# oviniciuscesar/Pseudo-Quadrature-Mirror-Filter

Measured on NVIDIA B200. Metric: PQMF analyze+inverse throughput (n_band=16), higher is better.
Workload: dtype f32

## Files before the change

pseudo-quadrature-mirror-filter_b200/csrc/hankel4.cuh:

```cuda
#pragma once
#include <cuda_fp16.h>
#include <cuda_runtime.h>
#include <math.h>
#include <stdint.h>
#include <string.h>

#include <atomic>

#include "half_io.cuh"
#include "hankel16.cuh"
#include "pcm.cuh"
#include "ptx.cuh"

namespace pqmf {

constexpr int kH4Workers = 256;
constexpr int kH4Threads = kH4Workers + 32;
constexpr int kH4SynWorkers = 288;
constexpr int kH4SynThreads = kH4SynWorkers + 32;
constexpr int kH4Rows = 128;
constexpr int kH4TileSamples = 64 * kH4Rows;
constexpr int kH4MaxPlaneRows = 144;
constexpr float kH4Res = 2048.0f;

__device__ __forceinline__ uint64_t umma_desc_sw128(uint32_t smem_addr) {
  uint64_t d = 0;
  d |= (uint64_t)((smem_addr & 0x3FFFFu) >> 4);
  d |= (uint64_t)1 << 16;
  d |= (uint64_t)(1024u >> 4) << 32;
  d |= (uint64_t)1 << 46;
  d |= (uint64_t)2 << 61;
  return d;
}
__device__ __forceinline__ uint32_t sw128_offset(uint32_t byte_lin) { return byte_lin ^ (((byte_lin >> 7) & 7u) << 4); }

struct H4Shape {
  int jlo, kt, ks;
  int rows, plane;
  int bank;
  int bytes;
// ... 37 lines not shown
}

__device__ __forceinline__ void split2_f16s(float a, float b, uint32_t& h1_bits, uint32_t& h2_bits) {
  const __half2 h1 = __floats2half2_rn(a, b);
  const float2 h1f = __half22float2(h1);
  const float2 r = __ffma2_rn(h1f, make_float2(-kH4Res, -kH4Res), __fmul2_rn(make_float2(a, b), make_float2(kH4Res, kH4Res)));
  const __half2 h2 = __floats2half2_rn(r.x, r.y);
  h1_bits = *reinterpret_cast<const uint32_t*>(&h1);
  h2_bits = *reinterpret_cast<const uint32_t*>(&h2);
}
__device__ __forceinline__ float2 h4_combine2(uint32_t d0a, uint32_t d0b, uint32_t d1a, uint32_t d1b) {
  const float2 t = __ffma2_rn(make_float2(__uint_as_float(d1a), __uint_as_float(d1b)), make_float2(1.0f / kH4Res, 1.0f / kH4Res),
                              make_float2(__uint_as_float(d0a), __uint_as_float(d0b)));
  constexpr float kInv = 1.0f / (float)(1 << kH16ScaleLog2);
  return __fmul2_rn(t, make_float2(kInv, kInv));
}

template <int N>
__device__ __forceinline__ void h4_tmem_ld(uint32_t taddr, uint32_t (&r)[N]) {
  static_assert(N == 2 || N == 4 || N == 8 || N == 16 || N == 32, "columns per load");
  if constexpr (N == 2) ptx::tmem_ld2(taddr, r);
  else if constexpr (N == 4) ptx::tmem_ld4(taddr, r);
  else if constexpr (N == 8) ptx::tmem_ld8(taddr, r);
  else if constexpr (N == 16) ptx::tmem_ld16(taddr, r);
  else ptx::tmem_ld32(taddr, r);
}

#ifdef PQMF_H4_TRACE
#define H4_STAMP(k) do { if (blockIdx.x == 0 && (tid & 31) == 0 && it < 64) p.trace[((size_t)it * 8 + warp) * 8 + (k)] = clock64(); } while (0)
#else
#define H4_STAMP(k) do { } while (0)
#endif

struct H4Smem {
  unsigned char *bank, *planes;
  uint64_t *pfull, *mma_bar, *bankfull;
  uint32_t* tmem_slot;
};
__device__ __forceinline__ H4Smem h4_carve(unsigned char* smem, const H4Shape& g) {
  H4Smem s;
  s.bank = smem;
  s.planes = smem + g.bank;
  s.pfull = reinterpret_cast<uint64_t*>(smem + g.bank + 4 * g.plane);
  s.mma_bar = s.pfull + 2;
  s.bankfull = s.mma_bar + 2;
  s.tmem_slot = reinterpret_cast<uint32_t*>(s.bankfull + 1);
  return s;
}

template <bool PAIR>
__device__ __forceinline__ uint32_t h4_prologue(const H4Smem& s, const H4Shape& g, const uint16_t* bank_images, uint32_t rank, int worker_warps,
                                                int tid) {
  const int warp = tid >> 5;
  ptx::grid_dep_launch();
  if (tid == 0) {
    for (int i = 0; i < 2; ++i) {
      ptx::mbar_init(&s.pfull[i], worker_warps * (PAIR ? 2 : 1));
      ptx::mbar_init(&s.mma_bar[i], 1);
    }
    ptx::mbar_init(s.bankfull, 1);
    ptx::fence_barrier_init();
    ptx::mbar_arrive_expect_tx(s.bankfull, (uint32_t)g.bank);
    ptx::bulk_g2s(s.bank, reinterpret_cast<const unsigned char*>(bank_images) + (size_t)rank * g.bank, (uint32_t)g.bank, s.bankfull);
  }
  if (warp == 0) {
    if constexpr (PAIR) {
      ptx::tmem_alloc_pair(s.tmem_slot, 256);
    } else {
      ptx::tmem_alloc(s.tmem_slot, 256);
      ptx::tmem_relinquish();
    }
  }
  ptx::tc_fence_before();
  __syncthreads();
  if constexpr (PAIR) ptx::cluster_sync_all();
  ptx::tc_fence_after();
  ptx::grid_dep_wait();
  return *s.tmem_slot;
}

template <bool PAIR>
__device__ __forceinline__ void h4_teardown(uint32_t tmem, int warp) {
  ptx::tc_fence_before();
  __syncthreads();
  if constexpr (PAIR) {
    ptx::cluster_sync_all();
    if (warp == 0) ptx::tmem_dealloc_pair(tmem, 256);
  } else {
    if (warp == 0) ptx::tmem_dealloc(tmem, 256);
  }
}

template <bool PAIR>
__device__ __forceinline__ void h4_issuer_loop(const H4Smem& s, const H4Shape& g, uint32_t tmem, unsigned n_iter, int pad_bytes, int tlo,
                                               int thi, unsigned it0 = 0) {
  const uint32_t bank_addr = ptx::smem_u32(s.bank), plane_addr = ptx::smem_u32(s.planes);
  for (unsigned it = it0; it < it0 + n_iter; ++it) {
    const int pb = (int)(it & 1);
    ptx::mbar_wait(&s.pfull[pb], (it >> 1) & 1);
    ptx::tc_fence_after();
    if (ptx::elect_one_sync()) {
      h4_issue_mmas<PAIR>(tmem + (uint32_t)(pb * 128), plane_addr + (2 * pb) * g.plane, plane_addr + (2 * pb + 1) * g.plane, bank_addr, g.ks,
                          pad_bytes, tlo, thi);
      if constexpr (PAIR) ptx::umma_pair_commit(&s.mma_bar[pb]);
      else ptx::umma_commit(&s.mma_bar[pb]);
    }
    __syncwarp();
  }
}

template <bool PAIR>
__device__ __forceinline__ void h4_publish(const H4Smem& s, uint32_t pfull_leader, unsigned it, int pb, int tid, unsigned it0 = 0, unsigned bank_phase = 0) {
  ptx::fence_proxy_async();
  ptx::tc_fence_before();
  __syncwarp();
  if ((tid & 31) == 0) {
    if (it == it0) ptx::mbar_wait(s.bankfull, bank_phase & 1);
    if constexpr (PAIR) ptx::mbar_arrive_cluster(pfull_leader + 8u * pb);
    else ptx::mbar_arrive(&s.pfull[pb]);
  }
}

struct H4AnalysisParams {
  const float* x;
  PcmIn in;
  float* y;
  const uint16_t* bank;
  long T, F;
  int off;
  int parity;
  int trim_lo, trim_hi;
  int accumulate;
  int keep_in_l2;
  H4Shape g;
  long tiles_per_row, n_tiles;
#ifdef PQMF_H4_TRACE
  long long* trace;
#endif
};

template <int M, bool PAIR, H4Io IO>
__global__ void __launch_bounds__(kH4Threads, 1) h4_analysis_kernel(H4AnalysisParams p) {
  constexpr bool PCM = IO == H4Io::PCM, HALF = h4_io_half(IO);
  constexpr int FR = 64 / M;
  constexpr int HB = M / 2;
  constexpr int NO = (kH4MaxPlaneRows * 8 + kH4Workers - 1) / kH4Workers;
  extern __shared__ __align__(1024) unsigned char h4_smem[];
  const H4Shape g = p.g;
  const H4Smem sm = h4_carve(h4_smem, g);
  const int tid = threadIdx.x, warp = tid >> 5;
  constexpr int kMmaWarp = kH4Workers / 32;
  const uint32_t rank = PAIR ? ptx::cluster_ctarank() : 0u;
  const uint32_t tmem = h4_prologue<PAIR>(sm, g, p.bank, rank, kH4Workers / 32, tid);
  const uint32_t pfull_leader = PAIR ? ptx::mapa_shared(ptx::smem_u32(sm.pfull), 0) : 0u;

  const unsigned tpr = (unsigned)p.tiles_per_row;
  const unsigned step_b = gridDim.x / tpr, step_c = gridDim.x % tpr;
  unsigned b = blockIdx.x / tpr, c = blockIdx.x % tpr;
  const unsigned first_tile = PAIR ? (blockIdx.x & ~1u) : blockIdx.x;
  const unsigned n_iter = (unsigned)((p.n_tiles - first_tile + gridDim.x - 1) / gridDim.x);
  const unsigned n_rows = (unsigned)(p.n_tiles / p.tiles_per_row);
#ifdef PQMF_H4_TRACE
  long long cta_c0 = clock64(), cta_t0;
  asm volatile("mov.u64 %0, %%globaltimer;" : "=l"(cta_t0));
#endif

  if (warp == kMmaWarp) {
    if (rank == 0) h4_issuer_loop<PAIR>(sm, g, tmem, n_iter, 0, p.trim_lo, p.trim_hi);
  } else {
    const int n_octs = g.rows * 8;
    float x0[NO][8];
    auto load_window = [&](unsigned bb, unsigned cc) {
      const long s0 = (long)cc * kH4TileSamples + g.jlo - p.off;
      const float* xrow = p.x + (size_t)bb * p.T;
      const uint16_t* xhrow = reinterpret_cast<const uint16_t*>(p.x) + (size_t)bb * p.T;
#pragma unroll
      for (int r = 0; r < NO; ++r) {
        const int o = tid + kH4Workers * r;
        const long s = s0 + 8L * o;
        if (bb < n_rows && o < n_octs && s >= 0 && s < p.T) {
          if constexpr (PCM) {
            pcm_load8_raw(p.in, bb, s, p.T, x0[r]);
          } else if constexpr (HALF) {
            const float4 raw = ptx::ldg128_na(reinterpret_cast<const float4*>(xhrow + s));
            x0[r][0] = raw.x; x0[r][1] = raw.y; x0[r][2] = raw.z; x0[r][3] = raw.w;
          } else {
            ptx::ldg256_na(xrow + s, x0[r]);
          }
        } else {
#pragma unroll
          for (int e = 0; e < 8; ++e) x0[r][e] = 0.f;
        }
      }
    };
    auto convert = [&](int pb, unsigned bb, unsigned cc) {
      unsigned char* p1 = sm.planes + (2 * pb) * g.plane;
      unsigned char* p2 = p1 + g.plane;
#pragma unroll
      for (int r = 0; r < NO; ++r) {
        const int o = tid + kH4Workers * r;
        if (o < n_octs) {
          if constexpr (PCM) {
            const long s = (long)cc * kH4TileSamples + g.jlo - p.off + 8L * o;
            if (bb < n_rows && s >= 0 && s < p.T) pcm_convert8(p.in, bb, x0[r]);
          }
          if constexpr (HALF) h4_widen8<IO>(x0[r]);
          uint4 a, bq;
          split2_f16s(x0[r][0], x0[r][1], a.x, bq.x);
          split2_f16s(x0[r][2], x0[r][3], a.y, bq.y);
          split2_f16s(x0[r][4], x0[r][5], a.z, bq.z);
          split2_f16s(x0[r][6], x0[r][7], a.w, bq.w);
          const uint32_t off = sw128_offset((uint32_t)o * 16u);
          *reinterpret_cast<uint4*>(p1 + off) = a;
          *reinterpret_cast<uint4*>(p2 + off) = bq;
        }
      }
    };
    auto advance = [&](unsigned& bb, unsigned& cc) {
      bb += step_b;
      cc += step_c;
      if (cc >= tpr) {
        cc -= tpr;
        ++bb;
      }
    };
    auto epilogue = [&](unsigned bb, unsigned cc, int dbuf) {
      const int i = tid & 127, hb = tid >> 7;
      const uint32_t taddr = tmem + ((uint32_t)((warp & 3) * 32) << 16) + (uint32_t)(dbuf * 128 + HB * hb);
      const long n = ((long)cc * kH4Rows + i) * FR;
      uint32_t r0[FR][HB], r1[FR][HB];
#pragma unroll
      for (int dl = 0; dl < FR; ++dl) {
        h4_tmem_ld<HB>(taddr + dl * M, r0[dl]);
        h4_tmem_ld<HB>(taddr + 64 + dl * M, r1[dl]);
      }
      ptx::tmem_ld_wait();
      float v[FR][HB];
#pragma unroll
      for (int dl = 0; dl < FR; ++dl) {
        const uint32_t flip = (((FR > 1 ? dl : (int)(n & 1)) + p.parity) & 1) == 0 ? 0x80000000u : 0u;
#pragma unroll
        for (int kk = 0; kk < HB; kk += 2) {
          const float2 t = h4_combine2(r0[dl][kk], r0[dl][kk + 1], r1[dl][kk], r1[dl][kk + 1]);
          v[dl][kk] = t.x;
          v[dl][kk + 1] = __uint_as_float(__float_as_uint(t.y) ^ flip);
        }
      }
      if constexpr (HALF) {
        uint16_t* yp = reinterpret_cast<uint16_t*>(p.y) + ((size_t)bb * M + HB * hb) * p.F + n;
        if (n + FR - 1 < p.F && (p.F % (FR >= 8 ? 8 : FR)) == 0) {
#pragma unroll
          for (int kk = 0; kk < HB; ++kk) {
            uint16_t* q = yp + (size_t)kk * p.F;
            if constexpr (FR >= 8) {
#pragma unroll
              for (int d8 = 0; d8 < FR; d8 += 8) {
// ... 29 lines not shown
          for (int kk = 0; kk < HB; ++kk)
#pragma unroll
            for (int dl = 0; dl < FR; ++dl) prev[dl][kk] = __ldcs(yp + (size_t)kk * p.F + dl);
#pragma unroll
          for (int kk = 0; kk < HB; ++kk)
#pragma unroll
            for (int dl = 0; dl < FR; ++dl) v[dl][kk] += prev[dl][kk];
        }
#pragma unroll
        for (int kk = 0; kk < HB; ++kk) {
          float* q = yp + (size_t)kk * p.F;
          if constexpr (FR >= 4) {
#pragma unroll
            for (int d4 = 0; d4 < FR; d4 += 4) {
              const float4 w = make_float4(v[d4][kk], v[d4 + 1][kk], v[d4 + 2][kk], v[d4 + 3][kk]);
              if (p.keep_in_l2) *reinterpret_cast<float4*>(q + d4) = w;
              else __stcs(reinterpret_cast<float4*>(q + d4), w);
            }
          } else if constexpr (FR == 2) {
            __stcs(reinterpret_cast<float2*>(q), make_float2(v[0][kk], v[1][kk]));
          } else {
            __stcs(q, v[0][kk]);
          }
        }
      } else {
#pragma unroll
        for (int kk = 0; kk < HB; ++kk)
#pragma unroll
          for (int dl = 0; dl < FR; ++dl)
            if (n + dl < p.F) yp[(size_t)kk * p.F + dl] = v[dl][kk] + (p.accumulate ? yp[(size_t)kk * p.F + dl] : 0.f);
      }
    };

    unsigned b1 = b, c1 = c;
    advance(b1, c1);
    load_window(b, c);
    unsigned prev_b = 0, prev_c = 0;
    for (unsigned it = 0; it < n_iter; ++it) {
      const int pb = (int)(it & 1);
      H4_STAMP(0);
      convert(pb, b, c);
      H4_STAMP(1);
      h4_publish<PAIR>(sm, pfull_leader, it, pb, tid);
      if (it + 1 < n_iter) load_window(b1, c1);
      H4_STAMP(2);
      if (it > 0) {
        ptx::mbar_wait(&sm.mma_bar[(it - 1) & 1], ((it - 1) >> 1) & 1);
        ptx::tc_fence_after();
        if (prev_b < n_rows) epilogue(prev_b, prev_c, (int)((it - 1) & 1));
      }
      H4_STAMP(5);
      prev_b = b;
      prev_c = c;
      b = b1;
      c = c1;
      advance(b1, c1);
    }
    ptx::mbar_wait(&sm.mma_bar[(n_iter - 1) & 1], ((n_iter - 1) >> 1) & 1);
    ptx::tc_fence_after();
    if (prev_b < n_rows) epilogue(prev_b, prev_c, (int)((n_iter - 1) & 1));
  }
#ifdef PQMF_H4_TRACE
  __syncthreads();
  if (tid == 0) {
    long long t1;
    asm volatile("mov.u64 %0, %%globaltimer;" : "=l"(t1));
    p.trace[64 * 64 + 2 * blockIdx.x] = clock64() - cta_c0;
    p.trace[64 * 64 + 2 * blockIdx.x + 1] = t1 - cta_t0;
  }
#endif
  h4_teardown<PAIR>(tmem, warp);
}

struct H4SynthesisParams {
  const float* s;
  float* out;
  int16_t* pcm_out;
  int C;
  int duo;
  const uint16_t* bank;
  long F;
  int o;
  int parity;
  int trim_lo, trim_hi;
  int accumulate;
  int reverse;
  H4Shape g;
  long tiles_per_row, n_tiles;
#ifdef PQMF_H4_TRACE
  long long* trace;
#endif
};

template <int M, bool PAIR, H4Io IO>
__global__ void __launch_bounds__(kH4SynThreads, 1) h4_synthesis_kernel(H4SynthesisParams p) {
  constexpr bool PCM = IO == H4Io::PCM, HALF = h4_io_half(IO);
  constexpr int FR = 64 / M;
  constexpr int NBG = M >= 8 ? M / 8 : 1;
  constexpr int FPI = M >= 8 ? 4 : 32 / M;
  extern __shared__ __align__(1024) unsigned char h4s_smem[];
  const H4Shape g = p.g;
  const H4Smem sm = h4_carve(h4s_smem, g);
  const int tid = threadIdx.x, warp = tid >> 5;
  constexpr int kMmaWarp = kH4SynWorkers / 32;
  const uint32_t rank = PAIR ? ptx::cluster_ctarank() : 0u;
  const uint32_t tmem = h4_prologue<PAIR>(sm, g, p.bank, rank, kH4SynWorkers / 32, tid);
  const uint32_t pfull_leader = PAIR ? ptx::mapa_shared(ptx::smem_u32(sm.pfull), 0) : 0u;

  const unsigned tpr = (unsigned)p.tiles_per_row;
  const unsigned step_b = gridDim.x / tpr, step_c = gridDim.x % tpr;
  unsigned b = blockIdx.x / tpr, c = blockIdx.x % tpr;
  const unsigned first_tile = PAIR ? (blockIdx.x & ~1u) : blockIdx.x;
  const unsigned G = (PCM && p.duo) ? 2u : 1u;
  const unsigned n_iter = G * (unsigned)((p.n_tiles - first_tile + gridDim.x - 1) / gridDim.x);
  const unsigned n_rows = (unsigned)(p.n_tiles / p.tiles_per_row);

  const int ehi = (g.jlo + g.kt) / M - 1;
  const int pad = (p.o - ehi) & 3;
  const int nbase = p.o - ehi - pad;
  if (warp == kMmaWarp) {
    if (rank == 0) h4_issuer_loop<PAIR>(sm, g, tmem, n_iter, 2 * M * pad, p.trim_lo, p.trim_hi);
  } else {
    const int n_fq = (g.rows * FR + FPI - 1) / FPI;
    const int bg = tid / n_fq, fq = tid - bg * n_fq;
    const bool has_item = tid < n_fq * NBG;
    float4 v0[8];
    auto load4h = [&](const uint16_t* at, bool ok) {
      if (!ok) return make_float4(0.f, 0.f, 0.f, 0.f);
      const float2 raw = ptx::ldg64_na(at);
      return make_float4(raw.x, raw.y, 0.f, 0.f);
    };
    auto load_frames = [&](float4 (&v)[8], unsigned bb, unsigned cc, unsigned hh) {
      if (p.reverse && bb < n_rows) {
        bb = n_rows - 1 - bb;
        cc = tpr - 1 - cc;
      }
      const long n = (long)cc * (kH4Rows * FR) + nbase + FPI * fq;
      const bool live = bb < n_rows && has_item;
      const size_t row = (size_t)bb * G + hh;
      if constexpr (HALF) {
        if constexpr (M >= 8) {
          const uint16_t* sp = reinterpret_cast<const uint16_t*>(p.s) + (row * M + 8 * bg) * p.F + n;
          const bool ok = live && n >= 0 && n + 3 < p.F;
#pragma unroll
          for (int kk = 0; kk < 8; ++kk) v[kk] = load4h(sp + (size_t)kk * p.F, ok);
        } else {
          const uint16_t* sp = reinterpret_cast<const uint16_t*>(p.s) + row * M * p.F + n;
#pragma unroll
          for (int kk = 0; kk < 8; ++kk) {
            const int b4 = kk >> 1, h = kk & 1;
            v[kk] = load4h(sp + (size_t)b4 * p.F + 4 * h, live && n + 4 * h >= 0 && n + 4 * h + 3 < p.F);
          }
        }
      } else if constexpr (M >= 8) {
        const float* sp = p.s + (row * M + 8 * bg) * p.F + n;
        const bool ok = live && n >= 0 && n + 3 < p.F;
#pragma unroll
        for (int kk = 0; kk < 8; ++kk) v[kk] = ok ? ptx::ldg128_na(reinterpret_cast<const float4*>(sp + (size_t)kk * p.F)) : make_float4(0.f, 0.f, 0.f, 0.f);
      } else {
        const float* sp = p.s + row * M * p.F + n;
#pragma unroll
        for (int kk = 0; kk < 8; ++kk) {
          const int b4 = kk >> 1, h = kk & 1;
          const bool ok = live && n + 4 * h >= 0 && n + 4 * h + 3 < p.F;
          v[kk] = ok ? ptx::ldg128_na(reinterpret_cast<const float4*>(sp + (size_t)b4 * p.F + 4 * h)) : make_float4(0.f, 0.f, 0.f, 0.f);
        }
      }
    };
    const uint32_t flip_even = (p.parity & 1) ? 0u : 0x80000000u, flip_odd = flip_even ^ 0x80000000u;
    auto advance = [&](unsigned& bb, unsigned& cc) {
      bb += step_b;
      cc += step_c;
      if (cc >= tpr) {
        cc -= tpr;
        ++bb;
      }
    };
    auto convert = [&](const float4 (&v)[8], int pb) {
      if (!has_item) return;
      unsigned char* p1 = sm.planes + (2 * pb) * g.plane;
      auto comp = [](const float4& q, int c) { return c == 0 ? q.x : c == 1 ? q.y : c == 2 ? q.z : q.w; };
#pragma unroll
      for (int j = 0; j < 4; ++j) {
        float w[8];
        uint32_t o;
        if constexpr (M >= 8) {
          const uint32_t fl = (j & 1) ? flip_odd : flip_even;
#pragma unroll
          for (int kk = 0; kk < 8; ++kk) {
            const float t = comp(v[kk], j);
            w[kk] = (kk & 1) ? __uint_as_float(__float_as_uint(t) ^ fl) : t;
          }
          o = sw128_offset((uint32_t)(4 * fq + j) * (2u * M) + 16u * bg);
        } else {
#pragma unroll
          for (int kk = 0; kk < 8; ++kk) {
            const int b4 = kk & 3, odd = kk >> 2;
            const float t = comp(v[2 * b4 + (j >> 1)], 2 * (j & 1) + odd);
            w[kk] = (b4 & 1) ? __uint_as_float(__float_as_uint(t) ^ (odd ? flip_odd : flip_even)) : t;
          }
          o = sw128_offset((uint32_t)(8 * fq + 2 * j) * (2u * M));
        }
        uint4 h1, h2;
        split2_f16s(w[0], w[1], h1.x, h2.x);
        split2_f16s(w[2], w[3], h1.y, h2.y);
        split2_f16s(w[4], w[5], h1.z, h2.z);
        split2_f16s(w[6], w[7], h1.w, h2.w);
        *reinterpret_cast<uint4*>(p1 + o) = h1;
        *reinterpret_cast<uint4*>(p1 + g.plane + o) = h2;
      }
// ... 65 lines not shown
          }
          return;
        }
#pragma unroll
        for (int q = 0; q < 4; ++q)
          if (t0 + 64 * q + 7 < total) pcm_store8(p.pcm_out, p.C, (long)row, t0 + 64 * q, total, val[q]);
        return;
      }
      if constexpr (HALF) {
        uint16_t* op = reinterpret_cast<uint16_t*>(p.out) + row * total + t0;
#pragma unroll
        for (int q = 0; q < 4; ++q)
          if (t0 + 64 * q + 7 < total) {
            const uint4 w = make_uint4(h4_narrow2<IO>(val[q][0], val[q][1]), h4_narrow2<IO>(val[q][2], val[q][3]), h4_narrow2<IO>(val[q][4], val[q][5]),
                                       h4_narrow2<IO>(val[q][6], val[q][7]));
            __stcs(reinterpret_cast<uint4*>(op + (size_t)q * 64), w);
          }
        return;
      }
      float* op = p.out + row * total + t0;
#pragma unroll
      for (int q = 0; q < 4; ++q)
        if (t0 + 64 * q + 7 < total) {
          if (p.accumulate) {
            float prev[8];
            ptx::ldg256_cs(op + (size_t)q * 64, prev);
#pragma unroll
            for (int e = 0; e < 8; ++e) val[q][e] += prev[e];
          }
          ptx::stg256_cs(op + (size_t)q * 64, val[q]);
        }
    };

    auto next_visit = [&](unsigned& bb, unsigned& cc, unsigned& hh) {
      if (++hh == G) {
        hh = 0;
        advance(bb, cc);
      }
    };
    unsigned h = 0, b1 = b, c1 = c, h1 = 0;
    next_visit(b1, c1, h1);
    load_frames(v0, b, c, h);
    unsigned prev_b = 0, prev_c = 0, prev_h = 0;
    for (unsigned it = 0; it < n_iter; ++it) {
      const int pb = (int)(it & 1);
      H4_STAMP(0);
      if constexpr (HALF) {
        float4 w[8];
#pragma unroll
        for (int kk = 0; kk < 8; ++kk) w[kk] = h4_widen4<IO>(v0[kk]);
        convert(w, pb);
      } else {
        convert(v0, pb);
      }
      H4_STAMP(1);
      h4_publish<PAIR>(sm, pfull_leader, it, pb, tid);
      if (it + 1 < n_iter) load_frames(v0, b1, c1, h1);
      H4_STAMP(2);
      if (it > 0) {
        ptx::mbar_wait(&sm.mma_bar[(it - 1) & 1], ((it - 1) >> 1) & 1);
        ptx::tc_fence_after();
        if (warp < 8 && prev_b < n_rows) epilogue(prev_b, prev_c, prev_h, (int)((it - 1) & 1));
      }
      H4_STAMP(5);
      prev_b = b;
      prev_c = c;
      prev_h = h;
      b = b1;
      c = c1;
      h = h1;
      next_visit(b1, c1, h1);
    }
    ptx::mbar_wait(&sm.mma_bar[(n_iter - 1) & 1], ((n_iter - 1) >> 1) & 1);
    ptx::tc_fence_after();
    if (warp < 8 && prev_b < n_rows) epilogue(prev_b, prev_c, prev_h, (int)((n_iter - 1) & 1));
  }
  h4_teardown<PAIR>(tmem, warp);
}

struct H4Configured {
  std::atomic<int> bytes[64];
  H4Configured() {
    for (auto& b : bytes) b.store(0, std::memory_order_relaxed);
  }
};
inline int h4_sm_count(int dev) {
  static std::atomic<int> sm_count[64];
  int n = sm_count[dev].load(std::memory_order_relaxed);
  if (n == 0) {
    cudaDeviceGetAttribute(&n, cudaDevAttrMultiProcessorCount, dev);
    n = n > 0 ? n : 148;
    sm_count[dev].store(n, std::memory_order_relaxed);
  }
  return n;
}
template <typename Kern>
inline int h4_configure(Kern kern, int bytes, H4Configured& configured, int& sm_count_out) {
  int dev = 0;
  cudaGetDevice(&dev);
  dev &= 63;
  if (configured.bytes[dev].load(std::memory_order_acquire) < bytes) {
    cudaError_t e = cudaFuncSetAttribute(kern, cudaFuncAttributeMaxDynamicSharedMemorySize, bytes);
    if (e != cudaSuccess) return (int)e;
    int seen = configured.bytes[dev].load(std::memory_order_relaxed);
    while (seen < bytes && !configured.bytes[dev].compare_exchange_weak(seen, bytes, std::memory_order_release)) {
    }
  }
  sm_count_out = h4_sm_count(dev);
  return 0;
}

template <bool PAIR, typename Kern, typename Params>
inline int h4_launch(Kern kern, Params p, int B, long row_samples, int threads, H4Configured& configured, cudaStream_t st) {
  int sms = 0;
  if (!h4_shape_fits(p.g)) return -2;
  if (int e = h4_configure(kern, p.g.bytes, configured, sms)) return e;
  p.tiles_per_row = (row_samples + kH4TileSamples - 1) / kH4TileSamples;
  p.n_tiles = p.tiles_per_row * B;
  if (p.tiles_per_row >= (1L << 31) || p.n_tiles >= (1L << 40)) return -2;
  long grid = PAIR ? (sms & ~1) : sms;
  const long want = PAIR ? ((p.n_tiles + 1) & ~1L) : p.n_tiles;
  if (grid > want) grid = want;
  if constexpr (PAIR) {
    cudaLaunchConfig_t cfg = {};
    cfg.gridDim = dim3((unsigned)grid);
    cfg.blockDim = dim3((unsigned)threads);
    cfg.dynamicSmemBytes = (size_t)p.g.bytes;
    cfg.stream = st;
    cudaLaunchAttribute attr[2];
    attr[0].id = cudaLaunchAttributeClusterDimension;
    attr[0].val.clusterDim.x = 2;
    attr[0].val.clusterDim.y = 1;
    attr[0].val.clusterDim.z = 1;
    attr[1].id = cudaLaunchAttributeProgrammaticStreamSerialization;
    attr[1].val.programmaticStreamSerializationAllowed = 1;
    cfg.attrs = attr;
    cfg.numAttrs = 2;
    return (int)cudaLaunchKernelEx(&cfg, kern, p);
  } else {
    kern<<<(unsigned)grid, threads, p.g.bytes, st>>>(p);
    return (int)cudaGetLastError();
  }
}

template <int M, bool PAIR>
int h4_launch_analysis(H4AnalysisParams p, int B, cudaStream_t st, H4Io io = H4Io::F32) {
  static H4Configured configured[4];
  if (p.in.pcm != nullptr) io = H4Io::PCM;
  if (io != H4Io::F32) {
    if constexpr (PAIR) {
      switch (io) {
        case H4Io::PCM: return h4_launch<PAIR>(h4_analysis_kernel<M, PAIR, H4Io::PCM>, p, B, p.F * M, kH4Threads, configured[1], st);
        case H4Io::F16: return h4_launch<PAIR>(h4_analysis_kernel<M, PAIR, H4Io::F16>, p, B, p.F * M, kH4Threads, configured[2], st);
        case H4Io::BF16: return h4_launch<PAIR>(h4_analysis_kernel<M, PAIR, H4Io::BF16>, p, B, p.F * M, kH4Threads, configured[3], st);
        default: return -2;
      }
    } else {
      return -2;
    }
  }
  return h4_launch<PAIR>(h4_analysis_kernel<M, PAIR, H4Io::F32>, p, B, p.F * M, kH4Threads, configured[0], st);
}

template <int M, bool PAIR>
int h4_launch_synthesis(H4SynthesisParams p, int B, cudaStream_t st, H4Io io = H4Io::F32) {
  static H4Configured configured[4];
  if (p.pcm_out != nullptr) {
    if constexpr (PAIR) {
      p.duo = (p.C == 2 && B % 2 == 0) ? 1 : 0;
      return h4_launch<PAIR>(h4_synthesis_kernel<M, PAIR, H4Io::PCM>, p, p.duo ? B / 2 : B, p.F * M, kH4SynThreads, configured[1], st);
    } else {
      return -2;
    }
  }
  if (h4_io_half(io)) {
    if constexpr (PAIR) {
      if (io == H4Io::F16) return h4_launch<PAIR>(h4_synthesis_kernel<M, PAIR, H4Io::F16>, p, B, p.F * M, kH4SynThreads, configured[2], st);
      return h4_launch<PAIR>(h4_synthesis_kernel<M, PAIR, H4Io::BF16>, p, B, p.F * M, kH4SynThreads, configured[3], st);
    } else {
      return -2;
    }
  }
  return h4_launch<PAIR>(h4_synthesis_kernel<M, PAIR, H4Io::F32>, p, B, p.F * M, kH4SynThreads, configured[0], st);
}

inline void hankel4_build_banks(const float* hk , int M, int L, int jlo, int kt, uint16_t* img_analysis, uint16_t* img_synthesis) {
  auto bits = [](float v) {
    const __half h = __float2half_rn(v);
    uint16_t u;
    memcpy(&u, &h, 2);
    return u;
  };
  const int ks = (kt + 64 - M + 15) / 16, kp = 16 * ks;
  const int elo = jlo / M, ehi = (jlo + kt) / M - 1;
  const float sa = (float)(1 << kH16ScaleLog2), ss = (float)M * sa;
  for (int kc = 0; kc < kp / 8; ++kc)
    for (int row = 0; row < 128; ++row)
      for (int e8 = 0; e8 < 8; ++e8) {
        const int kap = 8 * kc + e8;
// ... 59 lines not shown
```

pseudo-quadrature-mirror-filter_b200/csrc/pqmf_b200.cu:

```cuda
#include "../../include/pqmf_b200.h"

#include <cuda_fp16.h>
#include <cuda_runtime.h>

#include <atomic>
#include <cmath>
#include <cstdio>
#include <cstdlib>
#include <cstring>
#include <mutex>
#include <thread>
#include <vector>

#include "direct_form.cuh"
#include "fast16.cuh"
#include "fast16_synth.cuh"
#include "hankel16.cuh"
#include "hankel4.cuh"
#include "hankel4_stream.cuh"

namespace {

std::atomic<unsigned long long> g_launches{0};

// ... 503 lines not shown
    }
    if (rc) break;
    check(cudaEventRecord(ws.kdone[slot], ks));
    prev.live = true;
    prev.slot = slot;
    prev.r0 = r0;
    prev.n = n;
  }
  if (prev.live && rc == PQMF_OK) copy_out(prev, ws.kst[prev.slot]);
  for (int i = 0; i < kHostSlots; ++i) {
    check(cudaStreamSynchronize(ws.st[i]));
    check(cudaStreamSynchronize(ws.kst[i]));
  }
  return rc;
}

}

extern "C" {

int pqmf_abi_version(void) { return PQMF_B200_ABI_VERSION; }

const char* pqmf_strerror(int code) {
  switch (code) {
    case PQMF_OK: return "ok";
    case PQMF_ERR_ARG: return "pqmf_b200: invalid argument (null pointer, bad size or misaligned buffer)";
    case PQMF_ERR_UNSUPPORTED: return "pqmf_b200: unsupported parameter combination";
    case PQMF_ERR_NO_DEVICE: return "pqmf_b200: no usable CUDA device (needs sm_100)";
    default: return code > 0 ? cudaGetErrorString((cudaError_t)code) : "pqmf_b200: unknown error";
  }
}

unsigned long long pqmf_launch_count(void) { return g_launches.load(); }

int pqmf_path_for(int M, int L, const float* tables, unsigned flags) {
  return (use_fast(M, L, tables, flags) || use_h4_family(M, L, tables, flags)) ? 1 : 0;
}

long pqmf_tables_numel(int M, int L) {
  if (pqmf::hankel16_supported(M, L)) return kH4PairOffset + 2L * kH4PairImageFloats;
  return h4_family(M, L) ? h4_tables_floats(M, L) : 0;
}

int pqmf_build_tables_f32(const float* hk_host, const float* h_host, int N, int M, int L, float* tables_host,
                          double* residual, unsigned* fast_flags) {
  if (!hk_host || !h_host || !tables_host || N <= 0 || N > L) return PQMF_ERR_ARG;
  if (!pqmf::hankel16_supported(M, L)) {
    if (!h4_family(M, L)) return PQMF_ERR_UNSUPPORTED;
    int first = L, last = -1;
    for (int k = 0; k < M; ++k)
      for (int j = 0; j < L; ++j)
        if (hk_host[(size_t)k * L + j] != 0.f) {
          first = j < first ? j : first;
          last = j > last ? j : last;
        }
    if (last < 0) return PQMF_ERR_UNSUPPORTED;
    const int al = M > 32 ? M : 32;
    int jlo = (first / al) * al, kt = ((last + al) / al) * al - jlo;
    auto fits = [&](int j0, int k0) {
      return pqmf::h4_shape_fits(pqmf::h4_shape(M, j0, k0, true, false)) && pqmf::h4_shape_fits(pqmf::h4_shape(M, j0, k0, true, true));
    };
    bool split = false;
    if (!fits(jlo, kt)) {
      if (kt % (2 * al) != 0) {
        if (jlo + kt + al <= L) kt += al;
        else if (jlo >= al) { jlo -= al; kt += al; }
// ... 458 lines not shown
```

pseudo-quadrature-mirror-filter_b200/csrc/ptx.cuh:

```cuda
#pragma once
#include <cuda_fp16.h>
#include <cuda_runtime.h>
#include <stdint.h>

namespace pqmf {
namespace ptx {

__device__ __forceinline__ uint32_t smem_u32(const void* p) { return (uint32_t)__cvta_generic_to_shared(p); }

__device__ __forceinline__ void mbar_init(uint64_t* bar, uint32_t count) {
  asm volatile("mbarrier.init.shared::cta.b64 [%0], %1;" ::"r"(smem_u32(bar)), "r"(count));
}
__device__ __forceinline__ void fence_barrier_init() { asm volatile("fence.mbarrier_init.release.cluster;" ::: "memory"); }
__device__ __forceinline__ void mbar_arrive_expect_tx(uint64_t* bar, uint32_t bytes) {
  asm volatile("mbarrier.arrive.expect_tx.shared::cta.b64 _, [%0], %1;" ::"r"(smem_u32(bar)), "r"(bytes) : "memory");
}
__device__ __forceinline__ void mbar_arrive(uint64_t* bar) {
  asm volatile("mbarrier.arrive.shared::cta.b64 _, [%0];" ::"r"(smem_u32(bar)) : "memory");
}
__device__ __forceinline__ bool mbar_try_wait(uint64_t* bar, uint32_t parity) {
  uint32_t ok;
  asm volatile(
      "{\n\t.reg .pred p;\n\t"
      "mbarrier.try_wait.parity.shared::cta.b64 p, [%1], %2, %3;\n\t"
// ... 132 lines not shown
  const uint32_t addr = smem_u32(bar);
  uint32_t done = 0;
  while (!done) {
    asm volatile(
        "{\n\t.reg .pred p;\n\t"
        "mbarrier.try_wait.parity.acquire.cluster.shared::cta.b64 p, [%1], %2;\n\t"
        "selp.u32 %0, 1, 0, p;\n\t}"
        : "=r"(done)
        : "r"(addr), "r"(parity)
        : "memory");
  }
}
__device__ __forceinline__ void tmem_alloc_pair(uint32_t* slot, uint32_t cols) {
  asm volatile("tcgen05.alloc.cta_group::2.sync.aligned.shared::cta.b32 [%0], %1;" ::"r"(smem_u32(slot)), "r"(cols) : "memory");
  asm volatile("tcgen05.relinquish_alloc_permit.cta_group::2.sync.aligned;" ::: "memory");
}
__device__ __forceinline__ void tmem_dealloc_pair(uint32_t addr, uint32_t cols) {
  asm volatile("tcgen05.dealloc.cta_group::2.sync.aligned.b32 %0, %1;" ::"r"(addr), "r"(cols) : "memory");
}
__device__ __forceinline__ void umma_pair_f16(uint32_t d_tmem, uint64_t a_desc, uint64_t b_desc, uint32_t idesc, bool accumulate) {
  asm volatile(
      "{\n\t.reg .pred p;\n\t"
      "setp.ne.b32 p, %4, 0;\n\t"
      "tcgen05.mma.cta_group::2.kind::f16 [%0], %1, %2, %3, p;\n\t}" ::"r"(d_tmem),
      "l"(a_desc), "l"(b_desc), "r"(idesc), "r"((uint32_t)accumulate)
      : "memory");
}
__device__ __forceinline__ void umma_pair_commit(uint64_t* bar) {
  asm volatile("tcgen05.commit.cta_group::2.mbarrier::arrive::one.shared::cluster.multicast::cluster.b64 [%0], %1;" ::"r"(smem_u32(bar)),
               "h"((uint16_t)3)
               : "memory");
}

__device__ __forceinline__ void grid_dep_wait() { asm volatile("griddepcontrol.wait;" ::: "memory"); }
__device__ __forceinline__ void grid_dep_launch() { asm volatile("griddepcontrol.launch_dependents;" ::: "memory"); }

__device__ __forceinline__ void stg256_cs(float* p, const float (&v)[8]) {
  asm volatile("st.global.cs.v8.f32 [%0], {%1,%2,%3,%4,%5,%6,%7,%8};" ::"l"(p), "f"(v[0]), "f"(v[1]), "f"(v[2]), "f"(v[3]), "f"(v[4]),
               "f"(v[5]), "f"(v[6]), "f"(v[7])
               : "memory");
}
__device__ __forceinline__ void ldg256_cs(const float* p, float (&v)[8]) {
  asm volatile("ld.global.cs.v8.f32 {%0,%1,%2,%3,%4,%5,%6,%7}, [%8];"
               : "=f"(v[0]), "=f"(v[1]), "=f"(v[2]), "=f"(v[3]), "=f"(v[4]), "=f"(v[5]), "=f"(v[6]), "=f"(v[7])
               : "l"(p));
}

__device__ __forceinline__ void ldg256_na(const float* p, float (&v)[8]) {
  asm volatile("ld.global.nc.L1::no_allocate.v8.f32 {%0,%1,%2,%3,%4,%5,%6,%7}, [%8];"
               : "=f"(v[0]), "=f"(v[1]), "=f"(v[2]), "=f"(v[3]), "=f"(v[4]), "=f"(v[5]), "=f"(v[6]), "=f"(v[7])
               : "l"(p));
}
__device__ __forceinline__ float4 ldg128_na(const float4* p) {
  float4 v;
  asm volatile("ld.global.nc.L1::no_allocate.v4.f32 {%0,%1,%2,%3}, [%4];" : "=f"(v.x), "=f"(v.y), "=f"(v.z), "=f"(v.w) : "l"(p));
  return v;
}
__device__ __forceinline__ float2 ldg64_na(const void* p) {
  float2 v;
  asm volatile("ld.global.nc.L1::no_allocate.v2.f32 {%0,%1}, [%2];" : "=f"(v.x), "=f"(v.y) : "l"(p));
  return v;
}

__device__ __forceinline__ float4 ldg128_cg(const float4* p) {
  float4 v;
  asm volatile("ld.global.cg.v4.f32 {%0,%1,%2,%3}, [%4];" : "=f"(v.x), "=f"(v.y), "=f"(v.z), "=f"(v.w) : "l"(p) : "memory");
// ... 18 lines not shown
```

Baseline: 257,600.

## Replace static tile striding with dynamic atomic work claiming in H4 kernels

Swaps the fixed grid-stride tile assignment in the paired-CTA analysis and synthesis kernels for a dynamic scheduler. The first two units per cluster stay static, and later units are claimed through a global atomic counter and broadcast to both CTAs via cluster shared memory slots. The aim is to balance tail work across SMs when some CTAs start late or run slow. The cost is an atomic per iteration, spin-waits on shared memory slots, and host-side counter allocation per stream. It also adds optional boundary-trace instrumentation that is compiled out by default.

```diff
diff --git a/pseudo-quadrature-mirror-filter_b200/csrc/hankel4.cuh b/pseudo-quadrature-mirror-filter_b200/csrc/hankel4.cuh
--- a/pseudo-quadrature-mirror-filter_b200/csrc/hankel4.cuh
+++ b/pseudo-quadrature-mirror-filter_b200/csrc/hankel4.cuh
@@ -6,6 +6,9 @@
 #include <string.h>
 
 #include <atomic>
+#include <map>
+#include <mutex>
+#include <utility>
 
 #include "half_io.cuh"
 #include "hankel16.cuh"
@@ -109,10 +112,30 @@
 #define H4_STAMP(k) do { } while (0)
 #endif
 
+enum H4Bt { kBtEntry, kBtPrologue, kBtWaitDone, kBtFirstLoad, kBtFirstCommit, kBtLastStore, kBtExit, kBtInfo };
+#ifdef PQMF_H4_BOUNDARY_TRACE
+constexpr int kH4BtSlots = 64, kH4BtCtas = 160;
+__device__ unsigned long long h4_bt[kH4BtSlots][kH4BtCtas][8];
+__device__ __forceinline__ unsigned long long h4_gtimer() {
+  unsigned long long t;
+  asm volatile("mov.u64 %0, %%globaltimer;" : "=l"(t));
+  return t;
+}
+#define H4_BT(slot, k) do { if (blockIdx.x < kH4BtCtas && (slot) != ~0u) h4_bt[(slot) % kH4BtSlots][blockIdx.x][(k)] = h4_gtimer(); } while (0)
+#define H4_BT_INFO(slot, syn) do { if (blockIdx.x < kH4BtCtas) { unsigned smid_; asm volatile("mov.u32 %0, %%smid;" : "=r"(smid_)); \
+  h4_bt[(slot) % kH4BtSlots][blockIdx.x][kBtInfo] = smid_ | ((PAIR ? ptx::cluster_ctarank() : 0u) << 16) | ((unsigned)(syn) << 17); } } while (0)
+#define H4_BT_SLOT , p.bt_slot
+#else
+#define H4_BT_SLOT
+#define H4_BT(slot, k) do { } while (0)
+#define H4_BT_INFO(slot, syn) do { } while (0)
+#endif
+
 struct H4Smem {
   unsigned char *bank, *planes;
   uint64_t *pfull, *mma_bar, *bankfull;
   uint32_t* tmem_slot;
+  uint64_t* units;
 };
 __device__ __forceinline__ H4Smem h4_carve(unsigned char* smem, const H4Shape& g) {
   H4Smem s;
@@ -122,12 +145,13 @@
   s.mma_bar = s.pfull + 2;
   s.bankfull = s.mma_bar + 2;
   s.tmem_slot = reinterpret_cast<uint32_t*>(s.bankfull + 1);
+  s.units = s.bankfull + 2;
   return s;
 }
 
 template <bool PAIR>
 __device__ __forceinline__ uint32_t h4_prologue(const H4Smem& s, const H4Shape& g, const uint16_t* bank_images, uint32_t rank, int worker_warps,
-                                                int tid) {
+                                                int tid, unsigned bt_slot = ~0u) {
   const int warp = tid >> 5;
   ptx::grid_dep_launch();
   if (tid == 0) {
@@ -136,6 +160,7 @@
       ptx::mbar_init(&s.mma_bar[i], 1);
     }
     ptx::mbar_init(s.bankfull, 1);
+    for (int i = 0; i < 4; ++i) s.units[i] = 0;
     ptx::fence_barrier_init();
     ptx::mbar_arrive_expect_tx(s.bankfull, (uint32_t)g.bank);
     ptx::bulk_g2s(s.bank, reinterpret_cast<const unsigned char*>(bank_images) + (size_t)rank * g.bank, (uint32_t)g.bank, s.bankfull);
@@ -152,7 +177,9 @@
   __syncthreads();
   if constexpr (PAIR) ptx::cluster_sync_all();
   ptx::tc_fence_after();
+  if (tid == 0) H4_BT(bt_slot, kBtPrologue);
   ptx::grid_dep_wait();
+  if (tid == 0) H4_BT(bt_slot, kBtWaitDone);
   return *s.tmem_slot;
 }
 
@@ -168,11 +195,11 @@
   }
 }
 
-template <bool PAIR>
-__device__ __forceinline__ void h4_issuer_loop(const H4Smem& s, const H4Shape& g, uint32_t tmem, unsigned n_iter, int pad_bytes, int tlo,
-                                               int thi, unsigned it0 = 0) {
+template <bool PAIR, class More>
+__device__ __forceinline__ void h4_issuer_loop_while(const H4Smem& s, const H4Shape& g, uint32_t tmem, More more, int pad_bytes, int tlo,
+                                                     int thi, unsigned it0 = 0, unsigned bt_slot = ~0u) {
   const uint32_t bank_addr = ptx::smem_u32(s.bank), plane_addr = ptx::smem_u32(s.planes);
-  for (unsigned it = it0; it < it0 + n_iter; ++it) {
+  for (unsigned it = it0; more(it); ++it) {
     const int pb = (int)(it & 1);
     ptx::mbar_wait(&s.pfull[pb], (it >> 1) & 1);
     ptx::tc_fence_after();
@@ -181,9 +208,69 @@
                           pad_bytes, tlo, thi);
       if constexpr (PAIR) ptx::umma_pair_commit(&s.mma_bar[pb]);
       else ptx::umma_commit(&s.mma_bar[pb]);
+      if (it == it0) H4_BT(bt_slot, kBtFirstCommit);
     }
     __syncwarp();
   }
+}
+template <bool PAIR>
+__device__ __forceinline__ void h4_issuer_loop(const H4Smem& s, const H4Shape& g, uint32_t tmem, unsigned n_iter, int pad_bytes, int tlo,
+                                               int thi, unsigned it0 = 0) {
+  h4_issuer_loop_while<PAIR>(s, g, tmem, [=](unsigned it) { return it < it0 + n_iter; }, pad_bytes, tlo, thi, it0);
+}
+
+struct H4Sched {
+  unsigned group, groups, n_units;
+  unsigned* counter;
+  uint32_t units_own, units_peer;
+  uint32_t units_local;
+  bool claimer, alive;
+  unsigned pending;
+
+  __device__ __forceinline__ unsigned unit(unsigned i) const {
+    if (i < 2 || counter == nullptr) {
+      const unsigned u = group + i * groups;
+      return u < n_units ? u : ~0u;
+    }
+    unsigned long long v;
+    do {
+      v = ptx::ld_volatile_shared_u64(units_local + 8u * (i & 3));
+    } while ((unsigned)(v >> 32) != i);
+    return (unsigned)v;
+  }
+  __device__ __forceinline__ bool claiming() const { return counter != nullptr && claimer && alive; }
+  __device__ __forceinline__ void claim_issue() {
+    if (claiming()) pending = atomicAdd(counter, 1u);
+  }
+  __device__ __forceinline__ void claim_post(unsigned i) {
+    if (!claiming()) return;
+    const unsigned dyn = n_units > 2 * groups ? n_units - 2 * groups : 0u;
+    if (pending == dyn + groups - 1) atomicExch(counter, 0u);
+    unsigned u = 2 * groups + pending;
+    if (u >= n_units) {
+      u = ~0u;
+      alive = false;
+    }
+    const unsigned long long v = ((unsigned long long)(i + 2) << 32) | u;
+    ptx::st_cluster_u64(units_own + 8u * ((i + 2) & 3), v);
+    if (units_peer != units_own) ptx::st_cluster_u64(units_peer + 8u * ((i + 2) & 3), v);
+  }
+};
+template <bool PAIR>
+__device__ __forceinline__ H4Sched h4_sched(const H4Smem& s, unsigned* counter, long n_tiles, uint32_t rank) {
+  H4Sched q;
+  constexpr unsigned W = PAIR ? 2 : 1;
+  q.group = blockIdx.x / W;
+  q.groups = gridDim.x / W;
+  q.n_units = (unsigned)((n_tiles + W - 1) / W);
+  q.counter = counter;
+  q.units_local = ptx::smem_u32(s.units);
+  q.units_own = PAIR ? ptx::mapa_shared(q.units_local, rank) : q.units_local;
+  q.units_peer = PAIR ? ptx::mapa_shared(q.units_local, rank ^ 1u) : q.units_local;
+  q.claimer = rank == 0 && threadIdx.x == 0;
+  q.alive = true;
+  q.pending = 0;
+  return q;
 }
 
 template <bool PAIR>
@@ -209,10 +296,14 @@
   int trim_lo, trim_hi;
   int accumulate;
   int keep_in_l2;
+  unsigned* claim;
   H4Shape g;
   long tiles_per_row, n_tiles;
 #ifdef PQMF_H4_TRACE
   long long* trace;
+#endif
+#ifdef PQMF_H4_BOUNDARY_TRACE
+  unsigned bt_slot;
 #endif
 };
 
@@ -228,22 +319,28 @@
   const int tid = threadIdx.x, warp = tid >> 5;
   constexpr int kMmaWarp = kH4Workers / 32;
   const uint32_t rank = PAIR ? ptx::cluster_ctarank() : 0u;
-  const uint32_t tmem = h4_prologue<PAIR>(sm, g, p.bank, rank, kH4Workers / 32, tid);
+  if (tid == 0) {
+    H4_BT(p.bt_slot, kBtEntry);
+    H4_BT_INFO(p.bt_slot, 0);
+  }
+  const uint32_t tmem = h4_prologue<PAIR>(sm, g, p.bank, rank, kH4Workers / 32, tid H4_BT_SLOT);
   const uint32_t pfull_leader = PAIR ? ptx::mapa_shared(ptx::smem_u32(sm.pfull), 0) : 0u;
 
   const unsigned tpr = (unsigned)p.tiles_per_row;
-  const unsigned step_b = gridDim.x / tpr, step_c = gridDim.x % tpr;
-  unsigned b = blockIdx.x / tpr, c = blockIdx.x % tpr;
-  const unsigned first_tile = PAIR ? (blockIdx.x & ~1u) : blockIdx.x;
-  const unsigned n_iter = (unsigned)((p.n_tiles - first_tile + gridDim.x - 1) / gridDim.x);
   const unsigned n_rows = (unsigned)(p.n_tiles / p.tiles_per_row);
+  H4Sched sched = h4_sched<PAIR>(sm, p.claim, p.n_tiles, rank);
+  auto tile_of = [&](unsigned u, unsigned& bb, unsigned& cc) {
+    const unsigned t = u * (PAIR ? 2u : 1u) + rank;
+    bb = t / tpr;
+    cc = t - bb * tpr;
+  };
 #ifdef PQMF_H4_TRACE
   long long cta_c0 = clock64(), cta_t0;
   asm volatile("mov.u64 %0, %%globaltimer;" : "=l"(cta_t0));
 #endif
 
   if (warp == kMmaWarp) {
-    if (rank == 0) h4_issuer_loop<PAIR>(sm, g, tmem, n_iter, 0, p.trim_lo, p.trim_hi);
+    if (rank == 0) h4_issuer_loop_while<PAIR>(sm, g, tmem, [&](unsigned it) { return sched.unit(it) != ~0u; }, 0, p.trim_lo, p.trim_hi, 0u H4_BT_SLOT);
   } else {
     const int n_octs = g.rows * 8;
     float x0[NO][8];
@@ -291,14 +388,6 @@
           *reinterpret_cast<uint4*>(p1 + off) = a;
           *reinterpret_cast<uint4*>(p2 + off) = bq;
         }
-      }
-    };
-    auto advance = [&](unsigned& bb, unsigned& cc) {
-      bb += step_b;
-      cc += step_c;
-      if (cc >= tpr) {
-        cc -= tpr;
-        ++bb;
       }
     };
     auto epilogue = [&](unsigned bb, unsigned cc, int dbuf) {
@@ -394,33 +483,41 @@
       }
     };
 
-    unsigned b1 = b, c1 = c;
-    advance(b1, c1);
+    unsigned b, c, b1 = 0, c1 = 0;
+    tile_of(sched.unit(0), b, c);
+    if (tid == 0) H4_BT(p.bt_slot, kBtFirstLoad);
     load_window(b, c);
-    unsigned prev_b = 0, prev_c = 0;
-    for (unsigned it = 0; it < n_iter; ++it) {
+    unsigned prev_b = 0, prev_c = 0, it = 0;
+    for (;; ++it) {
       const int pb = (int)(it & 1);
+      sched.claim_issue();
       H4_STAMP(0);
       convert(pb, b, c);
       H4_STAMP(1);
       h4_publish<PAIR>(sm, pfull_leader, it, pb, tid);
-      if (it + 1 < n_iter) load_window(b1, c1);
+      const unsigned u1 = sched.unit(it + 1);
+      if (u1 != ~0u) {
+        tile_of(u1, b1, c1);
+        load_window(b1, c1);
+      }
       H4_STAMP(2);
       if (it > 0) {
         ptx::mbar_wait(&sm.mma_bar[(it - 1) & 1], ((it - 1) >> 1) & 1);
         ptx::tc_fence_after();
         if (prev_b < n_rows) epilogue(prev_b, prev_c, (int)((it - 1) & 1));
       }
+      sched.claim_post(it);
       H4_STAMP(5);
       prev_b = b;
       prev_c = c;
       b = b1;
       c = c1;
-      advance(b1, c1);
-    }
-    ptx::mbar_wait(&sm.mma_bar[(n_iter - 1) & 1], ((n_iter - 1) >> 1) & 1);
+      if (u1 == ~0u) break;
+    }
+    ptx::mbar_wait(&sm.mma_bar[it & 1], (it >> 1) & 1);
     ptx::tc_fence_after();
-    if (prev_b < n_rows) epilogue(prev_b, prev_c, (int)((n_iter - 1) & 1));
+    if (prev_b < n_rows) epilogue(prev_b, prev_c, (int)(it & 1));
+    if (tid == 0) H4_BT(p.bt_slot, kBtLastStore);
   }
 #ifdef PQMF_H4_TRACE
   __syncthreads();
@@ -432,6 +529,7 @@
   }
 #endif
   h4_teardown<PAIR>(tmem, warp);
+  if (tid == 0) H4_BT(p.bt_slot, kBtExit);
 }
 
 struct H4SynthesisParams {
@@ -447,10 +545,14 @@
   int trim_lo, trim_hi;
   int accumulate;
   int reverse;
+  unsigned* claim;
   H4Shape g;
   long tiles_per_row, n_tiles;
 #ifdef PQMF_H4_TRACE
   long long* trace;
+#endif
+#ifdef PQMF_H4_BOUNDARY_TRACE
+  unsigned bt_slot;
 #endif
 };
 
@@ -466,22 +568,30 @@
   const int tid = threadIdx.x, warp = tid >> 5;
   constexpr int kMmaWarp = kH4SynWorkers / 32;
   const uint32_t rank = PAIR ? ptx::cluster_ctarank() : 0u;
-  const uint32_t tmem = h4_prologue<PAIR>(sm, g, p.bank, rank, kH4SynWorkers / 32, tid);
+  if (tid == 0) {
+    H4_BT(p.bt_slot, kBtEntry);
+    H4_BT_INFO(p.bt_slot, 1);
+  }
+  const uint32_t tmem = h4_prologue<PAIR>(sm, g, p.bank, rank, kH4SynWorkers / 32, tid H4_BT_SLOT);
   const uint32_t pfull_leader = PAIR ? ptx::mapa_shared(ptx::smem_u32(sm.pfull), 0) : 0u;
 
   const unsigned tpr = (unsigned)p.tiles_per_row;
-  const unsigned step_b = gridDim.x / tpr, step_c = gridDim.x % tpr;
-  unsigned b = blockIdx.x / tpr, c = blockIdx.x % tpr;
-  const unsigned first_tile = PAIR ? (blockIdx.x & ~1u) : blockIdx.x;
   const unsigned G = (PCM && p.duo) ? 2u : 1u;
-  const unsigned n_iter = G * (unsigned)((p.n_tiles - first_tile + gridDim.x - 1) / gridDim.x);
   const unsigned n_rows = (unsigned)(p.n_tiles / p.tiles_per_row);
+  H4Sched sched = h4_sched<PAIR>(sm, G == 1 ? p.claim : nullptr, p.n_tiles, rank);
+  auto tile_of = [&](unsigned u, unsigned& bb, unsigned& cc) {
+    const unsigned t = u * (PAIR ? 2u : 1u) + rank;
+    bb = t / tpr;
+    cc = t - bb * tpr;
+  };
 
   const int ehi = (g.jlo + g.kt) / M - 1;
   const int pad = (p.o - ehi) & 3;
   const int nbase = p.o - ehi - pad;
   if (warp == kMmaWarp) {
-    if (rank == 0) h4_issuer_loop<PAIR>(sm, g, tmem, n_iter, 2 * M * pad, p.trim_lo, p.trim_hi);
+    if (rank == 0)
+      h4_issuer_loop_while<PAIR>(sm, g, tmem, [&](unsigned it) { return sched.unit(it / G) != ~0u; }, 2 * M * pad, p.trim_lo, p.trim_hi,
+                                 0u H4_BT_SLOT);
   } else {
     const int n_fq = (g.rows * FR + FPI - 1) / FPI;
     const int bg = tid / n_fq, fq = tid - bg * n_fq;
@@ -530,14 +640,6 @@
       }
     };
     const uint32_t flip_even = (p.parity & 1) ? 0u : 0x80000000u, flip_odd = flip_even ^ 0x80000000u;
-    auto advance = [&](unsigned& bb, unsigned& cc) {
-      bb += step_b;
-      cc += step_c;
-      if (cc >= tpr) {
-        cc -= tpr;
-        ++bb;
-      }
-    };
     auto convert = [&](const float4 (&v)[8], int pb) {
       if (!has_item) return;
       unsigned char* p1 = sm.planes + (2 * pb) * g.plane;
@@ -669,18 +771,14 @@
         }
     };
 
-    auto next_visit = [&](unsigned& bb, unsigned& cc, unsigned& hh) {
-      if (++hh == G) {
-        hh = 0;
-        advance(bb, cc);
-      }
-    };
-    unsigned h = 0, b1 = b, c1 = c, h1 = 0;
-    next_visit(b1, c1, h1);
+    unsigned b, c, h = 0, b1 = 0, c1 = 0, h1 = 0;
+    tile_of(sched.unit(0), b, c);
+    if (tid == 0) H4_BT(p.bt_slot, kBtFirstLoad);
     load_frames(v0, b, c, h);
-    unsigned prev_b = 0, prev_c = 0, prev_h = 0;
-    for (unsigned it = 0; it < n_iter; ++it) {
+    unsigned prev_b = 0, prev_c = 0, prev_h = 0, it = 0;
+    for (;; ++it) {
       const int pb = (int)(it & 1);
+      sched.claim_issue();
       H4_STAMP(0);
       if constexpr (HALF) {
         float4 w[8];
@@ -692,13 +790,19 @@
       }
       H4_STAMP(1);
       h4_publish<PAIR>(sm, pfull_leader, it, pb, tid);
-      if (it + 1 < n_iter) load_frames(v0, b1, c1, h1);
+      const unsigned u1 = sched.unit((it + 1) / G);
+      if (u1 != ~0u) {
+        tile_of(u1, b1, c1);
+        h1 = (it + 1) % G;
+        load_frames(v0, b1, c1, h1);
+      }
       H4_STAMP(2);
       if (it > 0) {
         ptx::mbar_wait(&sm.mma_bar[(it - 1) & 1], ((it - 1) >> 1) & 1);
         ptx::tc_fence_after();
         if (warp < 8 && prev_b < n_rows) epilogue(prev_b, prev_c, prev_h, (int)((it - 1) & 1));
       }
+      sched.claim_post(it);
       H4_STAMP(5);
       prev_b = b;
       prev_c = c;
@@ -706,13 +810,15 @@
       b = b1;
       c = c1;
       h = h1;
-      next_visit(b1, c1, h1);
-    }
-    ptx::mbar_wait(&sm.mma_bar[(n_iter - 1) & 1], ((n_iter - 1) >> 1) & 1);
+      if (u1 == ~0u) break;
+    }
+    ptx::mbar_wait(&sm.mma_bar[it & 1], (it >> 1) & 1);
     ptx::tc_fence_after();
-    if (warp < 8 && prev_b < n_rows) epilogue(prev_b, prev_c, prev_h, (int)((n_iter - 1) & 1));
+    if (warp < 8 && prev_b < n_rows) epilogue(prev_b, prev_c, prev_h, (int)(it & 1));
+    if (tid == 0) H4_BT(p.bt_slot, kBtLastStore);
   }
   h4_teardown<PAIR>(tmem, warp);
+  if (tid == 0) H4_BT(p.bt_slot, kBtExit);
 }
 
 struct H4Configured {
@@ -747,11 +853,49 @@
   return 0;
 }
 
+inline unsigned* h4_claim_counter(cudaStream_t st) {
+  cudaStreamCaptureStatus cap = cudaStreamCaptureStatusNone;
+  unsigned long long sid = 0;
+  int dev = 0;
+  if (cudaStreamIsCapturing(st, &cap) != cudaSuccess || cap != cudaStreamCaptureStatusNone || cudaStreamGetId(st, &sid) != cudaSuccess ||
+      cudaGetDevice(&dev) != cudaSuccess) {
+    (void)cudaGetLastError();
+    return nullptr;
+  }
+  constexpr int kWords = 128, kStride = 32;
+  static std::mutex mutex;
+  static std::map<std::pair<int, unsigned long long>, unsigned*> words;
+  static std::map<int, std::pair<unsigned*, int>> chunk;
+  std::lock_guard<std::mutex> lock(mutex);
+  const auto key = std::make_pair(dev, sid);
+  const auto found = words.find(key);
+  if (found != words.end()) return found->second;
+  auto& ch = chunk[dev];
+  if (ch.first == nullptr || ch.second == kWords) {
+    unsigned* fresh = nullptr;
+    const size_t bytes = sizeof(unsigned) * kWords * kStride;
+    if (cudaMalloc(&fresh, bytes) != cudaSuccess) {
+      (void)cudaGetLastError();
+      return nullptr;
+    }
+    if (cudaMemsetAsync(fresh, 0, bytes, st) != cudaSuccess || cudaStreamSynchronize(st) != cudaSuccess) {
+      (void)cudaGetLastError();
+      cudaFree(fresh);
+      return nullptr;
+    }
+    ch = std::make_pair(fresh, 0);
+  }
+  unsigned* w = ch.first + (size_t)kStride * ch.second++;
+  words[key] = w;
+  return w;
+}
+
 template <bool PAIR, typename Kern, typename Params>
 inline int h4_launch(Kern kern, Params p, int B, long row_samples, int threads, H4Configured& configured, cudaStream_t st) {
   int sms = 0;
   if (!h4_shape_fits(p.g)) return -2;
   if (int e = h4_configure(kern, p.g.bytes, configured, sms)) return e;
+  p.claim = PAIR ? h4_claim_counter(st) : nullptr;
   p.tiles_per_row = (row_samples + kH4TileSamples - 1) / kH4TileSamples;
   p.n_tiles = p.tiles_per_row * B;
   if (p.tiles_per_row >= (1L << 31) || p.n_tiles >= (1L << 40)) return -2;
@@ -780,9 +924,16 @@
   }
 }
 
+#ifdef PQMF_H4_BOUNDARY_TRACE
+inline std::atomic<unsigned> h4_bt_launches{0};
+#endif
+
 template <int M, bool PAIR>
 int h4_launch_analysis(H4AnalysisParams p, int B, cudaStream_t st, H4Io io = H4Io::F32) {
   static H4Configured configured[4];
+#ifdef PQMF_H4_BOUNDARY_TRACE
+  p.bt_slot = h4_bt_launches.fetch_add(1);
+#endif
   if (p.in.pcm != nullptr) io = H4Io::PCM;
   if (io != H4Io::F32) {
     if constexpr (PAIR) {
@@ -802,6 +953,9 @@
 template <int M, bool PAIR>
 int h4_launch_synthesis(H4SynthesisParams p, int B, cudaStream_t st, H4Io io = H4Io::F32) {
   static H4Configured configured[4];
+#ifdef PQMF_H4_BOUNDARY_TRACE
+  p.bt_slot = h4_bt_launches.fetch_add(1);
+#endif
   if (p.pcm_out != nullptr) {
     if constexpr (PAIR) {
       p.duo = (p.C == 2 && B % 2 == 0) ? 1 : 0;
diff --git a/pseudo-quadrature-mirror-filter_b200/csrc/pqmf_b200.cu b/pseudo-quadrature-mirror-filter_b200/csrc/pqmf_b200.cu
--- a/pseudo-quadrature-mirror-filter_b200/csrc/pqmf_b200.cu
+++ b/pseudo-quadrature-mirror-filter_b200/csrc/pqmf_b200.cu
@@ -559,6 +559,13 @@
 }
 
 unsigned long long pqmf_launch_count(void) { return g_launches.load(); }
+
+#ifdef PQMF_H4_BOUNDARY_TRACE
+unsigned pqmf_h4_boundary_trace(unsigned long long* dst) {
+  if (dst == nullptr || cudaDeviceSynchronize() != cudaSuccess || cudaMemcpyFromSymbol(dst, pqmf::h4_bt, sizeof(pqmf::h4_bt)) != cudaSuccess) return 0;
+  return pqmf::h4_bt_launches.load();
+}
+#endif
 
 int pqmf_path_for(int M, int L, const float* tables, unsigned flags) {
   return (use_fast(M, L, tables, flags) || use_h4_family(M, L, tables, flags)) ? 1 : 0;
diff --git a/pseudo-quadrature-mirror-filter_b200/csrc/ptx.cuh b/pseudo-quadrature-mirror-filter_b200/csrc/ptx.cuh
--- a/pseudo-quadrature-mirror-filter_b200/csrc/ptx.cuh
+++ b/pseudo-quadrature-mirror-filter_b200/csrc/ptx.cuh
@@ -188,6 +188,15 @@
                : "memory");
 }
 
+__device__ __forceinline__ void st_cluster_u64(uint32_t cluster_addr, unsigned long long v) {
+  asm volatile("st.relaxed.cluster.shared::cluster.u64 [%0], %1;" ::"r"(cluster_addr), "l"(v) : "memory");
+}
+__device__ __forceinline__ unsigned long long ld_volatile_shared_u64(uint32_t smem_addr) {
+  unsigned long long v;
+  asm volatile("ld.volatile.shared.u64 %0, [%1];" : "=l"(v) : "r"(smem_addr) : "memory");
+  return v;
+}
+
 __device__ __forceinline__ void grid_dep_wait() { asm volatile("griddepcontrol.wait;" ::: "memory"); }
 __device__ __forceinline__ void grid_dep_launch() { asm volatile("griddepcontrol.launch_dependents;" ::: "memory"); }
 
```

Result: slower. 234,500, median of 6 (-9.0%).
